# cita-cloud/consensus_overlord

Hardware: AMD Instinct MI355X
Metric: BLS12-381 vote verifications/sec (batch 4096) at 1/2/4/8 MI355X vs host blst (higher is better)
Workload: dtype u32; 1 GPU; config3: 4096 distinct-message precommit votes per GPU, RLC batch verify; batch_per_gpu=4096, global_batch=4096, parallelism=single GPU

## Files before the change

### consensus_overlord_amd/_lib.py

```python
from __future__ import annotations

import ctypes
import os

_HERE = os.path.dirname(os.path.abspath(__file__))
LIB_PATH = os.environ.get("OVH_LIBPATH") or os.path.join(_HERE, "libovhip.so")

_u8p = ctypes.c_char_p
_sz = ctypes.c_size_t
_szp = ctypes.POINTER(ctypes.c_size_t)
_vp = ctypes.c_void_p

SIGNATURES = [
    ("ovh_create", _vp, [ctypes.c_int, _u8p, _sz, ctypes.c_uint32]),
    ("ovh_create_multi", _vp, [ctypes.POINTER(ctypes.c_int), ctypes.c_int, _u8p, _sz, ctypes.c_uint32]),
    ("ovh_multi_peer_matrix", ctypes.c_int, [_vp, _u8p, _sz]),
    ("ovh_destroy", None, [_vp]),
    ("ovh_device_count", ctypes.c_int, [_vp]),
    ("ovh_stream", _vp, [_vp]),
    ("ovh_sm3", ctypes.c_int, [_u8p, _sz, _u8p]),
    ("ovh_sm3_batch", ctypes.c_int, [_vp, _sz, _vp, _vp, _vp]),
    ("ovh_sm3_batch_device", ctypes.c_int, [_vp, _sz, _vp, _vp, _vp]),
    ("ovh_check_blocks", ctypes.c_int, [_vp, _sz, _vp, _vp, _vp, _vp, _vp, _vp, _vp]),
    ("ovh_vote_digests_device", ctypes.c_int, [_vp, _sz, _vp, _vp, _vp, _vp, _vp, _vp]),
# ... 21 lines not shown
    ("ovh_verify_batch_device", ctypes.c_int, [_vp, _sz, _vp, _vp, _vp, _vp]),
    ("ovh_batch_partial_device", ctypes.c_int, [_vp, _sz, _vp, _vp, _vp, _vp, _vp, _vp]),
    ("ovh_combine_partials_device", ctypes.c_int, [_vp, _sz, _vp, ctypes.POINTER(ctypes.c_int32)]),
    ("ovh_batch_fallback_device", ctypes.c_int, [_vp, _sz, _vp]),
    ("ovh_verify_batch_device_async", ctypes.c_int, [_vp, _sz, _vp, _vp, _vp, _vp]),
    ("ovh_verify_samemsg_device_async", ctypes.c_int, [_vp, _sz, _vp, _vp, _vp, _vp]),
    ("ovh_vote_spans", ctypes.c_int, [_vp, ctypes.POINTER(ctypes.c_float), _sz]),
    ("ovh_verify_batch_async", ctypes.c_int, [_vp, _sz, _vp, _vp, _vp, _vp]),
    ("ovh_batch_wait", ctypes.c_int, [_vp]),
    ("ovh_combine_partials_device_async", ctypes.c_int, [_vp, _sz, _vp, _sz, _vp, _vp]),
    ("ovh_stage_times", ctypes.c_int, [_vp, ctypes.POINTER(ctypes.c_float), _sz]),
    ("ovh_stage_name", ctypes.c_char_p, [ctypes.c_int]),
    ("ovh_vm_trace", ctypes.c_int, [_vp, ctypes.c_int, ctypes.POINTER(ctypes.c_uint64), _sz]),
    ("ovh_vm_clock", ctypes.c_int, [_vp, ctypes.POINTER(ctypes.c_uint64), _sz]),
    ("ovh_pool_log", ctypes.c_int, [_vp, ctypes.POINTER(ctypes.c_uint64), _sz]),
    ("ovh_diag_vm_occupancy", ctypes.c_int, [_vp, ctypes.c_int, _sz, ctypes.c_int, ctypes.c_int,
                                             ctypes.POINTER(ctypes.c_float)]),
    ("ovh_sign_batch_device", ctypes.c_int, [_vp, _sz, _vp, _vp, _vp]),
    ("ovh_sk_to_pk_batch_device", ctypes.c_int, [_vp, _sz, _vp, _vp]),
]

_lib = None


def load():
    global _lib
    if _lib is not None:
        return _lib
    if not os.path.exists(LIB_PATH):
        raise RuntimeError(
# ... 13 lines not shown
```

### consensus_overlord_amd/csrc/ovhip.hip

```cpp
#include <hip/hip_runtime.h>

#include <errno.h>
#include <stdlib.h>
#include <sys/random.h>
#include <sys/types.h>

#include <algorithm>
#include <atomic>
#include <deque>
#include <mutex>
#include <new>
#include <string>
#include <string.h>
#include <unordered_map>
#include <vector>

#include "../../include/ovhip.h"
#include "bls/verify.hpp"
#include "fpvm.hpp"
#include "keygen.hpp"
#include "proof.hpp"
#include "qc_segments.hpp"
#include "rlp.hpp"
#include "sm3.hpp"
#include "sm3_bulk.hpp"
#ifdef OVH_VM_PROGS
#include OVH_VM_PROGS
#else
#include <vm_progs.inc>
#endif
static_assert(VM_KZERO == ovh::vm::KZERO && VM_KTAB == ovh::vm::KTAB, "fixed constants (tools/fpvm/gen.py)");
#define VM_ASSERT_NO_INV(P) static_assert(!VM_##P##_HAS_INV, #P " has an inv op: it needs vm::run<SIDE, true>")
#define VM_ASSERT_INV(P) static_assert(VM_##P##_HAS_INV, #P " has no inv op: bind it to vm::run<SIDE, false>")
VM_ASSERT_NO_INV(MADD); VM_ASSERT_NO_INV(PADD); VM_ASSERT_NO_INV(G1PADD);
VM_ASSERT_NO_INV(HDBL1); VM_ASSERT_NO_INV(HDBL2); VM_ASSERT_NO_INV(HDBL4); VM_ASSERT_NO_INV(HDBL8); VM_ASSERT_NO_INV(HDBL16);
// ... 264 lines not shown
};

#define POOL_SEQR 16u
#define POOL_QW 16u
enum : uint32_t {
  PQ_CUR = 0,
  PQ_NPUB = POOL_QW,
  PQ_SLOTOF = 2 * POOL_QW,
  PQ_NANN = 3 * POOL_QW,
  PQ_DONE = 4 * POOL_QW,
  PQ_CLAIM = PQ_DONE + OVH_BATCH_SLOTS * POOL_QW,
  PQ_INFL = PQ_CLAIM + OVH_BATCH_SLOTS * POOL_QW,
  PQ_OCC = PQ_INFL + POOL_QW,
};
constexpr uint32_t POOL_OCC_N = 4096;
constexpr uint32_t PQ_WORDS = PQ_OCC + POOL_OCC_N / 2;
static_assert(POOL_SEQR > OVH_BATCH_SLOTS && POOL_SEQR / 2 <= POOL_QW, "pool queue layout");
#define POOL_IDLE_TICKS 2000ull
#define POOL_WAIT_TICKS 2000000ull

__device__ __forceinline__ uint32_t simd_key() {
  const uint32_t hw = __builtin_amdgcn_s_getreg((31 << 11) | 4);
  const uint32_t xcc = __builtin_amdgcn_s_getreg((3 << 11) | 20);
  return (xcc & 7u) << 9 | ((hw >> 13) & 3u) << 7 | ((hw >> 12) & 1u) << 6 | ((hw >> 8) & 15u) << 2 |
         ((hw >> 4) & 3u);
}
__device__ __forceinline__ uint32_t* pq_occ(uint64_t* q) { return reinterpret_cast<uint32_t*>(q + PQ_OCC); }
#define POOL_SPREAD_TICKS 20000ull

struct PoolBatch {
  uint64_t seq;
  uint32_t n, nq;
  uint32_t table;
  uint32_t has_idx;
  uint64_t seed, base;
  int32_t* codes;
  const uint32_t* planes;
  const uint32_t* flags;
  uint32_t pcap, cap;
  uint32_t* state;
  uint32_t* part0;
  const uint8_t* stage;
// ... 30 lines not shown
}

struct PoolArgs {
  uint64_t* q;
  const PoolBatch* descs;
  const uint4* pv_code;
  const uint32_t* pv_side;
  const uint4* pt_code;
  const uint32_t* pt_side;
  const uint4* fold_code;
  const uint32_t* cst;
  uint32_t* scr;
  uint64_t* wlog;
  uint64_t only;
  uint32_t nsimd;
  uint32_t skip_cu;
};

__device__ __forceinline__ uint64_t* pq_done(uint64_t* q, uint32_t slot) { return q + PQ_DONE + slot * POOL_QW; }
__device__ __forceinline__ uint64_t* pq_claim(uint64_t* q, uint32_t slot) { return q + PQ_CLAIM + slot * POOL_QW; }
__device__ __forceinline__ uint32_t* pq_slot_of(uint64_t* q) { return reinterpret_cast<uint32_t*>(q + PQ_SLOTOF); }
__device__ __forceinline__ uint64_t qld(const uint64_t* p) {
  return __hip_atomic_load(p, __ATOMIC_RELAXED, __HIP_MEMORY_SCOPE_AGENT);
}

__global__ __launch_bounds__(64) void k_pool_publish(PoolBatch b, uint32_t slot, uint64_t seq, uint64_t* q,
                                                     PoolBatch* descs) {
  if (threadIdx.x) return;
  b.seq = ~0ull;
  descs[slot] = b;
  __builtin_amdgcn_fence(__ATOMIC_RELEASE, "agent");
// ... 282 lines not shown
    pl[16 + 2 * quad] = pl_start | (uint64_t)simd_key() << 48 | (uint64_t)how << 60;
    pl[16 + 2 * quad + 1] = __builtin_amdgcn_s_memrealtime();
  }
  __builtin_amdgcn_fence(__ATOMIC_RELEASE, "agent");
  asm volatile("s_waitcnt vmcnt(0)" ::: "memory");
  if (threadIdx.x == 0) {
    __hip_atomic_fetch_add(pq_done(a.q, slot), 1ull, __ATOMIC_RELAXED, __HIP_MEMORY_SCOPE_AGENT);
    __hip_atomic_fetch_add(a.q + PQ_INFL, ~0ull, __ATOMIC_RELAXED, __HIP_MEMORY_SCOPE_AGENT);
    __hip_atomic_fetch_add(pq_occ(a.q) + simd_key(), ~0u, __ATOMIC_RELAXED, __HIP_MEMORY_SCOPE_AGENT);
  }
}

__global__ __launch_bounds__(64, 2) void k_vm_pool(PoolArgs a) {
  __builtin_amdgcn_s_setprio(2);
  extern __shared__ uint4 lds4[];
  if (a.skip_cu && ((simd_key() >> 2) & 0x7Fu) < a.skip_cu) return;
  uint32_t* lds = reinterpret_cast<uint32_t*>(lds4);
  load_consts(lds, a.cst, VM_NCONST);
  const uint64_t t_in = __builtin_amdgcn_s_memrealtime();
  vote_stagger();
  uint32_t nquads = 0, why = 0;
#pragma unroll 1
  for (;; ++nquads) {
    uint32_t slot = 0, quad = 0, how = 0;
    if (!pool_claim(a.q, a.descs, &slot, &quad, &why, a.only, a.nsimd, &how)) break;
    slot = uni(slot);
    quad = uni(quad) | uni(how) << 28;
    __builtin_amdgcn_fence(__ATOMIC_ACQUIRE, "agent");
    vote_quad(a, slot, quad, lds, uni(dget(&a.descs[slot].table)) != 0);
  }
  if (a.wlog && threadIdx.x == 0 && blockIdx.x < PLOG_WGS) {
    uint64_t* w = a.wlog + (size_t)blockIdx.x * PLOG_WG_WORDS;
    w[0] = t_in;
    w[1] = __builtin_amdgcn_s_memrealtime();
    w[2] = nquads;
    w[3] = why;
  }
}

__global__ __launch_bounds__(64) void k_pool_wait(uint64_t* q, uint32_t slot, uint32_t nq, uint64_t ticks,
                                                  uint32_t* err) {
  if (threadIdx.x) return;
  const uint64_t t0 = wall_clock64();
  while (__hip_atomic_load(pq_done(q, slot), __ATOMIC_RELAXED, __HIP_MEMORY_SCOPE_AGENT) < nq) {
    if (wall_clock64() - t0 > ticks) {
      __hip_atomic_store(err, 1u, __ATOMIC_RELAXED, __HIP_MEMORY_SCOPE_SYSTEM);
      return;
    }
    __builtin_amdgcn_s_sleep(32);
  }
}

// ... 1377 lines not shown
struct ovh_ctx {
  int device = 0;
  uint32_t flags = 0;
  hipStream_t stream = nullptr;
  hipStream_t fstream = nullptr, fstream2 = nullptr, fstream3 = nullptr;
  hipStream_t fstream4 = nullptr;
  uint32_t nfin = NFIN_STREAMS;
  hipStream_t xstream = nullptr;
  hipStream_t vstream[3] = {};
  hipStream_t hstream[4] = {};
  hipStream_t pool_st[3] = {};
  uint64_t* pool_q = nullptr;
  void* pool_desc = nullptr;
  uint32_t* pool_scr = nullptr;
  uint32_t pool_wgs = 0;
  uint32_t pool_grid0 = 0;
  uint32_t ncu = 256;
  uint32_t pool_rsv = 0;
  uint32_t pool_ncu = 256;
  uint64_t pool_seq = 0;
  uint32_t* pool_err = nullptr;
  uint64_t* plog = nullptr;
  uint64_t plog_seq[OVH_BATCH_SLOTS] = {};
  uint64_t plog_grids = 0;
  hipStream_t fs[OVH_BATCH_SLOTS] = {};
  hipEvent_t ev_front[OVH_BATCH_SLOTS] = {}, ev_back[OVH_BATCH_SLOTS] = {};
  hipEvent_t ev_x[4] = {};
  uint32_t* state_slot[OVH_BATCH_SLOTS] = {};
  uint32_t* red_slot[OVH_BATCH_SLOTS] = {};
  uint32_t *state_all = nullptr, *red_all = nullptr;
  uint8_t* pstage_all = nullptr;
  size_t state_w = 0, red_w = 0, pstage_b = 0;
  int32_t* grp_ok[OVH_BATCH_SLOTS] = {};
  uint32_t slot_n[OVH_BATCH_SLOTS] = {};
// ... 125 lines not shown
static_assert(LDS_VSAME8 <= 64 * 1024, "vsame8 LDS (default limit)");
static constexpr size_t LDS_H2G = ((size_t)SLOT_BASE_W + VM_SLICES * (size_t)H2G_STRIDE_W) * 4;
static constexpr size_t LDS_GMIL = ((size_t)SLOT_BASE_W + (size_t)VM_GMIL_NSLOTS * 12) * 4;
static_assert(LDS_VSAME <= 64 * 1024 && LDS_H2G <= 64 * 1024 && LDS_GMIL + 16 <= 64 * 1024, "same-message LDS");
static constexpr size_t LDS_PKDEC = ((size_t)SLOT_BASE_W + (64 / VM_PKDEC_W) * (size_t)PKDEC_STRIDE_W) * 4;
static_assert(LDS_PKDEC <= 64 * 1024 && VM_PKDEC_NIN == 2, "pkdec LDS / shape");
static constexpr size_t LDS_G1GRP = ((size_t)SLOT_BASE_W + (size_t)G1GRP_STRIDE_W) * 4;
static_assert(LDS_G1GRP <= 64 * 1024 && VM_G1GRP_NIN == 3, "g1grp LDS / shape");
static constexpr size_t LDS_GFIN = ((size_t)SLOT_BASE_W + (size_t)VM_GFIN_NSLOTS * 12) * 4;
static_assert(LDS_GFIN + 16 <= 64 * 1024, "gfin LDS");
constexpr size_t lds_granule(size_t b) { return (b + 1023) / 1024 * 1024; }
static constexpr size_t LDS_POOL = LDS_VOTE > LDS_VOTE_T ? LDS_VOTE : LDS_VOTE_T;
static_assert(8 * lds_granule(LDS_POOL) <= 160 * 1024, "eight pool workgroups per CU");
static_assert(VOTE_NSCR <= 4096 && VM_VOTE_NSLOTS <= 2048 && VM_VOTE_T_NSLOTS <= 2048,
              "side words: 12-bit scratch entries, 11-bit slots (fpvm.hpp side_spill)");
#ifndef POOL_HOLES_PER_8CU
#define POOL_HOLES_PER_8CU 8u
#endif
#define POOL_MAX_WGS 4096u
static_assert(FOLD_STRIDE_W <= VM_SLICES * VOTE_STRIDE_W && FOLD_STRIDE_W <= VM_SLICES * VOTE_T_STRIDE_W,
              "fused fold reuses the vote slots");

static int vm_upload(ovh_ctx* c, VmDev& d, const uint32_t* code, uint32_t nphases, uint32_t W, uint32_t NW,
                     const uint16_t* in, uint32_t nin, const uint16_t* out, uint32_t nout,
                     const uint32_t* side = nullptr) {
  const size_t words = (size_t)nphases * W * NW, pad = (size_t)vm::PREFETCH * W * NW;
  void *dc = nullptr, *di = nullptr, *dout = nullptr;
  HIPCHK(hipMalloc(&dc, (words + pad) * 4));
  c->vm_bufs.push_back(dc);
  HIPCHK(hipMemcpy(dc, code, words * 4, hipMemcpyHostToDevice));
  HIPCHK(hipMemset((uint32_t*)dc + words, 0, pad * 4));
  HIPCHK(hipMalloc(&di, nin * 2 + 2));
// ... 144 lines not shown
};

static const uint8_t DEFAULT_DST[] = "BLS_SIG_BLS12381G2_XMD:SHA-256_SSWU_RO_NUL_";

static uint32_t nblk(size_t n) { return (uint32_t)((n + WG - 1) / WG); }

static Slab region_F(ovh_ctx* c, int slot, int r) {
  return Slab{c->red_slot[slot] + (size_t)r * PART_PLANES * 12 * c->red_cap, c->red_cap};
}
static Slab region_S(ovh_ctx* c, int slot, int r) {
  return Slab{c->red_slot[slot] + (size_t)r * PART_PLANES * 12 * c->red_cap + (size_t)12 * 12 * c->red_cap,
              c->red_cap};
}

namespace {
struct ParkedStream {
  int device;
  int prio;
  hipStream_t s;
};
std::mutex g_park_mu;
std::vector<ParkedStream> g_parked;
}

static hipError_t stream_new(hipStream_t* s, int prio) {
  int dev = 0;
  const hipError_t e = hipGetDevice(&dev);
  if (e != hipSuccess) return e;
  {
    std::lock_guard<std::mutex> g(g_park_mu);
    for (size_t k = 0; k < g_parked.size(); ++k)
      if (g_parked[k].device == dev && g_parked[k].prio == prio) {
        *s = g_parked[k].s;
        g_parked.erase(g_parked.begin() + (ptrdiff_t)k);
        return hipSuccess;
      }
  }
  return hipStreamCreateWithPriority(s, hipStreamNonBlocking, prio);
}

static void stream_park(int device, hipStream_t s) {
  if (!s) return;
  (void)hipStreamSynchronize(s);
  int prio = 0;
  if (hipStreamGetPriority(s, &prio) != hipSuccess) return;
  std::lock_guard<std::mutex> g(g_park_mu);
  g_parked.push_back(ParkedStream{device, prio, s});
}

static int pool_failed(const ovh_ctx* c) {
  return c->pool_err && __atomic_load_n(c->pool_err, __ATOMIC_ACQUIRE) ? OVH_ERR_DEVICE : 0;
}

static int sync_all(ovh_ctx* c) {
  HIPCHK(hipStreamSynchronize(c->stream));
  HIPCHK(hipStreamSynchronize(c->fstream));
  HIPCHK(hipStreamSynchronize(c->fstream2));
  HIPCHK(hipStreamSynchronize(c->fstream3));
  if (c->fstream4) HIPCHK(hipStreamSynchronize(c->fstream4));
  for (hipStream_t s : {c->pool_st[0], c->pool_st[1], c->pool_st[2], c->vstream[0], c->vstream[1], c->vstream[2],
                        c->hstream[1], c->hstream[2], c->hstream[3]})
    if (s) HIPCHK(hipStreamSynchronize(s));
// ... 180 lines not shown
  b.part_cap = r0.cap;
  b.stage = ps;
  b.clk = table ? c->vm_vote_t.clk : c->vm_vote.clk;
  b.plog = c->plog ? c->plog + (size_t)(seq % PLOG_RING) * PLOG_WORDS : nullptr;
  c->plog_seq[slot] = seq;
  k_pool_publish<<<1, 64, 0, c->stream>>>(b, (uint32_t)slot, seq, c->pool_q, (PoolBatch*)c->pool_desc);
  if (b.plog) k_stamp<<<1, 64, 0, c->stream>>>(b.plog + PLOG_EV_PUB, seq);
  HIPCHK(hipEventRecord(c->ev_front[slot], c->stream));
  c->slot_n[slot] = n;
  c->last_n = n;
  const bool vev = (c->flags & OVH_FLAG_PROFILE) != 0;
  const uint32_t vk = c->vev_n % ovh_ctx::VEV_CAP;
  const uint32_t wgs = c->pool_wgs;
  PoolArgs pa;
  pa.only = ~0ull;
  pa.nsimd = 4 * c->pool_ncu;
  pa.skip_cu = c->pool_rsv / 8;
  shard = shard && !c->pool_rsv;
  pa.q = c->pool_q;
  pa.descs = (const PoolBatch*)c->pool_desc;
  pa.pv_code = c->vm_vote.code;
  pa.pv_side = c->vm_vote.side;
  pa.pt_code = c->vm_vote_t.code;
  pa.pt_side = c->vm_vote_t.side;
  pa.fold_code = c->vm_fold.code;
  pa.cst = c->vm_consts;
  for (uint32_t par = 0; launch && par < (shard ? c->shard_streams : 2u); ++par) {
    if (shard && par != (uint32_t)(seq % c->shard_streams)) continue;
    if (shard) pa.only = seq + c->shard_span;
    hipStream_t pst = c->pool_st[par];
    HIPCHK(hipStreamWaitEvent(pst, c->ev_front[slot], 0));
    if (par == 0 || shard) {
      if (c->flags & OVH_FLAG_PROFILE) HIPCHK(hipEventRecord(c->ev0[ST_VOTE], pst));
      if (vev) HIPCHK(hipEventRecord(c->vev0[vk], pst));
    }
    const uint32_t gw = shard ? 2 * wgs : par == 0 ? c->pool_grid0 : 2 * wgs - c->pool_grid0;
    pa.scr = c->pool_scr + (size_t)par * 2 * wgs * VM_SLICES * VOTE_NSCR * 12;
    pa.wlog = nullptr;
    if (c->plog) {
      uint64_t* g = c->plog + PLOG_GRID_BASE + (size_t)(c->plog_grids++ % PLOG_GRIDS) * (4 + PLOG_WGS * PLOG_WG_WORDS);
      k_grid_hdr<<<1, 64, 0, pst>>>(g, seq, par, gw);
      pa.wlog = g + 4;
    }
    k_vm_pool<<<gw, 64, LDS_POOL, pst>>>(pa);
    if (par == 1 || shard) {
      if (c->flags & OVH_FLAG_PROFILE) {
        HIPCHK(hipEventRecord(c->ev1[ST_VOTE], pst));
        c->ev_mask |= 1u << ST_VOTE;
      }
      if (vev) {
        HIPCHK(hipEventRecord(c->vev1[vk], pst));
// ... 403 lines not shown
  const uint32_t* head = pl.head;
  const uint32_t* pairs = pl.pairs;
  c->ev_mask = 0;
  uint64_t seed, base;
  CHK(draw_seed(c, &seed, &base));
  c->slot_seed[slot] = seed;
  c->slot_base[slot] = base;
  const hipStream_t fst = c->fs[slot];
  hipStream_t st = c->stream;
  if (one) {
    hipStream_t* pair = c->vstream;
    for (hipStream_t* v : {&pair[0], &pair[1]})
      if (!*v) {
        int lo = 0, hi = 0;
        (void)hipDeviceGetStreamPriorityRange(&lo, &hi);
        HIPCHK(stream_new(v, hi));
      }
    st = pair[c->pipe_k & 1];
  }
  if (!c->xstream) HIPCHK(stream_new(&c->xstream, 0));
  const uint32_t hk = one ? (uint32_t)(c->pipe_k % SM_H2G_STREAMS) : 0u;
  if (hk && !c->hstream[hk]) HIPCHK(stream_new(&c->hstream[hk], 0));
  const hipStream_t xs = one ? fst : c->xstream, hs = hk ? c->hstream[hk] : c->xstream;
  HIPCHK(hipEventRecord(c->ev_front[slot], c->stream));
  HIPCHK(hipStreamWaitEvent(hs, c->ev_front[slot], 0));
  HIPCHK(hipStreamWaitEvent(fst, c->ev_front[slot], 0));
  if (st != c->stream) HIPCHK(hipStreamWaitEvent(st, c->ev_front[slot], 0));
  {
    StageScope p(c, ST_H2F, hs);
    if (one) k_put_hash<<<1, 64, 0, hs>>>(*one, (uint8_t*)ghash);
    k_h2f<<<nblk(G), WG, 0, hs>>>(G, ghash, c->xmd, g);
    k_vm_h2g<<<(G + VM_SLICES - 1) / VM_SLICES, 64, LDS_H2G, hs>>>(G, c->vm_h2g, c->vm_consts, g, ghinf);
  }
  HIPCHK(hipEventRecord(c->ev_x[1], hs));
  HIPCHK(hipStreamWaitEvent(fst, c->ev_x[1], 0));
  const PkSrc tab{c->tab.planes, c->tab.cap, c->tab.flags, tidx};
  {
// ... 509 lines not shown
  if (!c) return nullptr;
  c->device = device;
  c->flags = flags;
  if (const char* e = getenv("OVH_SMALL_MAX")) c->small_max = (uint32_t)atoi(e);
  if (const char* e = getenv("OVH_SAMEMSG")) c->samemsg = atoi(e);
  if (const char* e = getenv("OVH_SHARD_SPAN")) c->shard_span = (uint32_t)atoi(e);
  if (const char* e = getenv("OVH_SHARD_STREAMS")) c->shard_streams = atoi(e) == 3 ? 3u : 2u;
  if (const char* e = getenv("OVH_NFIN")) c->nfin = atoi(e) == 3 ? 3u : atoi(e) == 2 ? 2u : NFIN_STREAMS;
  int ncu = 0;
  if (hipDeviceGetAttribute(&ncu, hipDeviceAttributeMultiprocessorCount, device) != hipSuccess || ncu <= 0) ncu = 256;
  if (flags & OVH_FLAG_POOL_RESERVE) {
    c->pool_rsv = 8;
    if (const char* e = getenv("OVH_POOL_RESERVE")) c->pool_rsv = (uint32_t)atoi(e);
    if (c->pool_rsv % 8 || c->pool_rsv > 64 || (uint32_t)ncu <= 2 * c->pool_rsv) c->pool_rsv = 0;
  }
  const uint32_t pncu = (uint32_t)ncu - c->pool_rsv;
  uint32_t holes = POOL_HOLES_PER_8CU;
  if (const char* e = c->pool_rsv ? getenv("OVH_POOL_PER_CU") : nullptr) holes = atoi(e) == 8 ? 0u : holes;
  c->pool_wgs = ((uint32_t)ncu * 8 - (uint32_t)ncu * holes / 8) / 2;
  if (c->pool_wgs > POOL_MAX_WGS) c->pool_wgs = POOL_MAX_WGS;
  c->pool_grid0 = std::min(4u * (uint32_t)ncu, 2 * c->pool_wgs - 1);
  c->ncu = (uint32_t)ncu;
  c->pool_ncu = pncu;
  if (!dst) {
    dst = DEFAULT_DST;
    dst_len = 43;
  }
  int lo = 0, hi = 0;
  (void)hipDeviceGetStreamPriorityRange(&lo, &hi);
  bool ok = xmd_build_templates(c->xmd, dst, dst_len) &&
            stream_new(&c->stream, 0) == hipSuccess &&
            stream_new(&c->fstream, lo) == hipSuccess &&
            stream_new(&c->fstream2, lo) == hipSuccess &&
            stream_new(&c->fstream3, lo) == hipSuccess &&
            (c->nfin < 4 || stream_new(&c->fstream4, lo) == hipSuccess) &&
            stream_new(&c->pool_st[0], hi) == hipSuccess &&
            stream_new(&c->pool_st[1], hi) == hipSuccess &&
            (c->shard_streams < 3 || stream_new(&c->pool_st[2], hi) == hipSuccess) &&
            hipMalloc(&c->part_out, (size_t)OVH_BATCH_SLOTS * 2 * 216 * 4) == hipSuccess && hipMalloc(&c->result, RES_WORDS * 4) == hipSuccess &&
            hipMemset(c->result, 0, RES_WORDS * 4) == hipSuccess &&
            hipMalloc(&c->pool_q, (size_t)PQ_WORDS * 8) == hipSuccess && hipMemset(c->pool_q, 0, (size_t)PQ_WORDS * 8) == hipSuccess &&
            hipMalloc(&c->pool_desc, sizeof(PoolBatch) * OVH_BATCH_SLOTS) == hipSuccess &&
            hipMemset(c->pool_desc, 0, sizeof(PoolBatch) * OVH_BATCH_SLOTS) == hipSuccess &&
            hipMalloc(&c->pool_scr, (size_t)2 * c->shard_streams * c->pool_wgs * VM_SLICES * VOTE_NSCR * 48) == hipSuccess &&
            hipHostMalloc((void**)&c->pool_err, 64, hipHostMallocCoherent | hipHostMallocMapped) == hipSuccess &&
            hipMalloc(&c->fin, (size_t)OVH_BATCH_SLOTS * FIN_STRIDE * 4) == hipSuccess && vm_init(c) == 0;
  if (ok) *c->pool_err = 0;
  if (ok && (flags & OVH_FLAG_VM_CLOCK))
    ok = hipMalloc(&c->plog, PLOG_TOTAL * 8) == hipSuccess && hipMemset(c->plog, 0, PLOG_TOTAL * 8) == hipSuccess;
  ok = ok && hipDeviceSynchronize() == hipSuccess;
  for (int k = 0; ok && k < OVH_BATCH_SLOTS; ++k) c->fs[k] = c->fstream;
  for (int k = 0; ok && k < OVH_BATCH_SLOTS; ++k)
    ok = hipEventCreateWithFlags(&c->ev_front[k], hipEventDisableTiming) == hipSuccess &&
         hipEventCreateWithFlags(&c->ev_back[k], hipEventDisableTiming) == hipSuccess;
  for (int k = 0; ok && k < 4; ++k) ok = hipEventCreateWithFlags(&c->ev_x[k], hipEventDisableTiming) == hipSuccess;
  for (int k = 0; ok && k < OVH_BATCH_SLOTS; ++k)
// ... 93 lines not shown
  for (int k = 0; k < OVH_BATCH_SLOTS; ++k) {
    for (int q = 0; q < 4; ++q)
      if (c->ev_m[k][q]) (void)hipEventDestroy(c->ev_m[k][q]);
    if (c->hst_h[k]) (void)hipHostFree(c->hst_h[k]);
    if (c->hst_d[k]) (void)hipFree(c->hst_d[k]);
  }
  if (c->mg) (void)hipFree(c->mg);
  for (int k = 0; k < OVH_NSTAGES; ++k) {
    if (c->ev0[k]) (void)hipEventDestroy(c->ev0[k]);
    if (c->ev1[k]) (void)hipEventDestroy(c->ev1[k]);
  }
  for (uint32_t k = 0; k < ovh_ctx::VEV_CAP; ++k) {
    if (c->vev0[k]) (void)hipEventDestroy(c->vev0[k]);
    if (c->vev1[k]) (void)hipEventDestroy(c->vev1[k]);
  }
  for (hipStream_t s : {c->stream, c->fstream, c->fstream2, c->fstream3, c->fstream4, c->xstream, c->vstream[0], c->vstream[1], c->vstream[2],
                        c->pool_st[0], c->pool_st[1], c->pool_st[2], c->hstream[1], c->hstream[2], c->hstream[3]})
    stream_park(c->device, s);
  if (c->pool_err) (void)hipHostFree(c->pool_err);
  delete c;
}

void ovh_destroy(ovh_ctx* c) {
  if (!c) return;
  for (ovh_ctx* s : c->sub) destroy_one(s);
  c->sub.clear();
  destroy_one(c);
}

int ovh_device_count(ovh_ctx* c) { return !c ? 0 : c->sub.empty() ? 1 : (int)c->sub.size(); }

int ovh_diag_vm_occupancy(ovh_ctx* c, int prog, size_t n, int reps, int streams, float* ms) {
  if (!c || !ms || n == 0 || n > (1u << 20) || reps < 1 || streams < 1 || streams > 2 || prog < 0 || prog > 2 ||
      (prog == 2 && reps > OVH_BATCH_SLOTS))
    return OVH_ERR_ARG;
  if (!c->sub.empty()) c = c->sub[0];
  std::lock_guard<std::mutex> g(c->mu);
  HIPCHK(hipSetDevice(c->device));
  CHK(ensure_cap(c, n));
  CHK(ensure_in(c, n * 180 + 64));
  CHK(sync_all(c));
  if (!c->xstream) HIPCHK(stream_new(&c->xstream, 0));
  HIPCHK(hipMemsetAsync(c->in_buf, 0, n * 180, c->stream));
  HIPCHK(hipStreamSynchronize(c->stream));
  const Slab s{c->state_slot[0], c->cap};
  int32_t* dc = (int32_t*)(c->in_buf + n * 176);
  const uint32_t N = (uint32_t)n;
  hipEvent_t e0, e1;
  HIPCHK(hipEventCreate(&e0));
  HIPCHK(hipEventCreate(&e1));
  HIPCHK(hipEventRecord(e0, c->stream));
  HIPCHK(hipStreamWaitEvent(c->xstream, e0, 0));
  for (int r = 0; r < reps; ++r) {
    if (prog == 0) {
      hipStream_t st = (streams == 2 && (r & 1)) ? c->xstream : c->stream;
      k_vm_vsame<false><<<(N + VM_SLICES - 1) / VM_SLICES, 64, LDS_VSAME, st>>>(N, 0, c->vm_vsame, c->vm_consts,
                                                                               c->in_buf + n * 128, PkSrc{}, c->in_buf,
// ... 43 lines not shown
  if (hipSetDevice(c->device) != hipSuccess || sync_all(c)) return -OVH_ERR_DEVICE;
  const VmDev* d = c->clk_table ? &c->vm_vote_t : &c->vm_vote;
  const size_t n = (size_t)2 * c->clk_wgs, k = max < n ? max : n;
  if (k && hipMemcpy(stamps, d->clk, k * 8, hipMemcpyDeviceToHost) != hipSuccess) return -OVH_ERR_DEVICE;
  return (int)n;
}

int ovh_pool_log(ovh_ctx* c, uint64_t* words, size_t max) {
  if (!c || (max && !words)) return -OVH_ERR_ARG;
  if (!c->sub.empty()) c = c->sub[0];
  if (!c->plog) return 0;
  std::lock_guard<std::mutex> g(c->mu);
  if (hipSetDevice(c->device) != hipSuccess || sync_all(c)) return -OVH_ERR_DEVICE;
  const size_t n = PLOG_TOTAL, k = max < n ? max : n;
  if (k && hipMemcpy(words, c->plog, k * 8, hipMemcpyDeviceToHost) != hipSuccess) return -OVH_ERR_DEVICE;
  return (int)n;
}

int ovh_stage_times(ovh_ctx* c, float* ms, size_t max) {
  if (!c || (!ms && max)) return -OVH_ERR_ARG;
  if (!c->sub.empty()) c = c->sub[0];
  if (!(c->flags & OVH_FLAG_PROFILE)) return 0;
  std::lock_guard<std::mutex> g(c->mu);
  if (hipSetDevice(c->device) != hipSuccess || sync_all(c)) return -OVH_ERR_DEVICE;
  const size_t n = max < OVH_NSTAGES ? max : OVH_NSTAGES;
  for (size_t k = 0; k < n; ++k) {
    ms[k] = 0.f;
    if (c->ev_mask & (1u << k))
      if (hipEventElapsedTime(&ms[k], c->ev0[k], c->ev1[k]) != hipSuccess) return -OVH_ERR_DEVICE;
  }
// ... 261 lines not shown
  CHK(stage_list(c, sigs, sig_lens, n, 0, &ds, &so, &sl, &used1));
  CHK(stage_list(c, pks, pk_lens, n, used1, &dp, &po, &pl, &used2));
  if (n && !compressed) {
    uint8_t* cs = c->in_buf + ((used2 + 15) & ~(size_t)15);
    uint64_t* co = (uint64_t*)(cs + (size_t)96 * n);
    k_canon_sig_list<<<nblk(n), WG, 0, c->stream>>>((uint32_t)n, ds, so, sl, cs, co);
    HIPCHK(hipGetLastError());
    ds = cs;
    so = co;
    used2 = (size_t)((uint8_t*)(co + n) - c->in_buf);
  }
  Slab pts{c->scr, c->scr_cap};
  Slab ppts{c->scr + (size_t)6 * 12 * c->scr_cap, c->scr_cap};
  if (n) {
    HIPCHK(hipEventRecord(c->ev_x[2], c->stream));
    if (!c->xstream) HIPCHK(stream_new(&c->xstream, 0));
    HIPCHK(hipStreamWaitEvent(c->xstream, c->ev_x[2], 0));
    bool keys48 = true;
    for (size_t i = 0; i < n; ++i) keys48 = keys48 && pk_lens[i] == 48;
    if (keys48) {
      constexpr uint32_t KSL = 64 / VM_PKDEC_W;
      k_vm_pkdec<<<(uint32_t)((n + KSL - 1) / KSL), 64, LDS_PKDEC, c->xstream>>>((uint32_t)n, c->vm_pkdec,
                                                                                c->vm_consts, dp, po, c->scr_pk);
    } else {
      k_parse_pk_list<<<nblk(n), WG, 0, c->xstream>>>((uint32_t)n, dp, po, pl, c->scr_pk, ppts);
    }
    HIPCHK(hipGetLastError());
    HIPCHK(hipEventRecord(c->ev_x[3], c->xstream));
    const int gc = (c->flags & OVH_FLAG_AGG_NO_GROUPCHECK) ? 0 : 1;
    constexpr uint32_t SL = 64 / VM_SIGCHK_W;
    k_vm_sigchk<<<(uint32_t)((n + SL - 1) / SL), 64, LDS_SIGCHK, c->stream>>>((uint32_t)n, c->vm_sigchk, c->vm_consts,
// ... 171 lines not shown
    uint8_t* dp;
    uint64_t *po, *pl;
    size_t used = 0;
    CHK(stage_list(c, pks, pk_lens, n, raw_base, &dp, &po, &pl, &used));
    uint8_t* rs = c->in_buf + used;
    if (agg_len) HIPCHK(hipMemcpyAsync(rs, agg_sig, agg_len, hipMemcpyHostToDevice, c->stream));
    k_canon_qc<<<nblk(n + 1), WG, 0, c->stream>>>((uint32_t)n, dp, po, pl, rs, (uint32_t)agg_len, d);
    HIPCHK(hipGetLastError());
  }
  HIPCHK(hipMemcpyAsync(d + n * 48 + 96, hash, 32, hipMemcpyHostToDevice, c->stream));
  int slot;
  CHK(take_slot(c, &slot));
  c->last_n = 0;
  Slab s{c->state_slot[slot], c->cap};
  HIPCHK(hipEventRecord(c->ev_x[2], c->stream));
  if (!c->xstream) HIPCHK(stream_new(&c->xstream, 0));
  HIPCHK(hipStreamWaitEvent(c->xstream, c->ev_x[2], 0));
  k_h2f<<<1, WG, 0, c->xstream>>>(1, d + n * 48 + 96, c->xmd, s);
  k_vm_qcpre<<<1, 64, LDS_QCPRE, c->xstream>>>(c->vm_qcpre, c->vm_consts, d + n * 48, s, qpf);
  HIPCHK(hipGetLastError());
  HIPCHK(hipEventRecord(c->ev_x[3], c->xstream));
  uint32_t* kflags = c->qt_buf + (size_t)3 * 12 * c->qt_cap;
  constexpr uint32_t PK_SL = 64 / VM_PKCHK_W;
  k_vm_pkchk<<<(uint32_t)((n + PK_SL - 1) / PK_SL), 64, LDS_PKCHK, c->stream>>>((uint32_t)n, c->vm_pkchk, c->vm_consts, d,
                                                                               Slab{c->qt_buf, c->qt_cap}, kflags);
  HIPCHK(hipGetLastError());
  std::vector<uint32_t> hf(n);
  HIPCHK(hipMemcpyAsync(hf.data(), kflags, n * 4, hipMemcpyDeviceToHost, c->stream));
  HIPCHK(hipStreamSynchronize(c->stream));
  uint32_t fl = 0;
  for (size_t i = 0; i < n; ++i) fl |= hf[i];
// ... 1062 lines not shown
```

### include/ovhip.h

```cpp
#ifndef OVHIP_H
#define OVHIP_H

#include <stddef.h>
#include <stdint.h>

#ifdef __cplusplus
extern "C" {
#endif

typedef struct ovh_ctx ovh_ctx;

#define OVH_OK 0
#define OVH_ERR_HASH_LEN 100
#define OVH_ERR_LEN_MISMATCH 101
#define OVH_ERR_PUBKEY 102
#define OVH_ERR_ARG 103
#define OVH_ERR_DEVICE 200
#define OVH_ERR_RNG 201

#define OVH_FLAG_AGG_NO_GROUPCHECK 0x1u
#define OVH_FLAG_PROFILE 0x2u
#define OVH_FLAG_VM_TRACE 0x4u
#define OVH_FLAG_TEST_RLC 0x8u
#define OVH_FLAG_SK_RAW 0x10u
// ... 86 lines not shown
int ovh_verify_batch_async(ovh_ctx* ctx, size_t n, const uint8_t* sigs, const uint8_t* hashes, const uint8_t* pks,
                           int32_t* codes);
int ovh_batch_wait(ovh_ctx* ctx);
int ovh_combine_partials_device_async(ovh_ctx* ctx, size_t k, const uint8_t* d_partials, size_t n,
                                      int32_t* d_codes, void* stream);

int ovh_stage_times(ovh_ctx* ctx, float* ms, size_t max);
const char* ovh_stage_name(int stage);
int ovh_vote_spans(ovh_ctx* ctx, float* ms, size_t max);

int ovh_vm_trace(ovh_ctx* ctx, int prog, uint64_t* stamps, size_t max);
int ovh_diag_vm_occupancy(ovh_ctx* ctx, int prog, size_t n, int reps, int streams, float* ms);
int ovh_vm_clock(ovh_ctx* ctx, uint64_t* stamps, size_t max);

int ovh_pool_log(ovh_ctx* ctx, uint64_t* words, size_t max);

int ovh_sign_batch_device(ovh_ctx* ctx, size_t n, const uint8_t* d_sks, const uint8_t* d_hashes, uint8_t* d_sigs);
int ovh_sk_to_pk_batch_device(ovh_ctx* ctx, size_t n, const uint8_t* d_sks, uint8_t* d_pks);

#ifdef __cplusplus
}
#endif

#endif
```

### overlord-hip/build.rs

```rust
use std::{env, path::PathBuf, process::Command};

fn main() {
    let manifest = PathBuf::from(env::var("CARGO_MANIFEST_DIR").unwrap());
    let src = env::var("OVHIP_SRC")
        .map(PathBuf::from)
        .unwrap_or_else(|_| manifest.join("../consensus_overlord_amd"));
    assert!(
        src.join("csrc/ovhip.hip").exists(),
        "libovhip sources not found at {} (set OVHIP_SRC)",
        src.display()
    );
    let hipcc = env::var("HIPCC").unwrap_or_else(|_| "/opt/rocm/bin/hipcc".into());
    let arch = env::var("OVHIP_ARCH").unwrap_or_else(|_| "gfx950".into());
    let out = PathBuf::from(env::var("OUT_DIR").unwrap());

    let gen = Command::new("python3")
        .arg(src.join("../tools/fpvm/gen.py"))
        .arg("--out")
        .arg(out.join("vm_progs.inc"))
        .status()
        .expect("python3 (tools/fpvm/gen.py)");
    assert!(gen.success(), "tools/fpvm/gen.py failed");

    let st = Command::new(&hipcc)
        .args(["-O3", "-std=c++17", "-fPIC", "-Wno-unused-result", "-shared"])
        .arg(format!("--offload-arch={arch}"))
        .arg(format!("-I{}", out.display()))
        .arg("-o")
        .arg(out.join("libovhip.so"))
        .arg(src.join("csrc/ovhip.hip"))
        .status()
        .expect("hipcc");
    assert!(st.success(), "hipcc --offload-arch={arch} failed");

    println!("cargo:rustc-link-search=native={}", out.display());
    println!("cargo:rustc-link-lib=dylib=ovhip");
    println!("cargo:rustc-link-arg=-Wl,-rpath,{}", out.display());
    for f in ["csrc/ovhip.hip", "csrc/fpvm.hpp", "csrc/msm.hpp", "csrc/keygen.hpp", "csrc/rlp.hpp", "csrc/sm3.hpp", "csrc/sm3_bulk.hpp", "csrc/proof.hpp", "csrc/qc.hpp", "csrc/bls"] {
        println!("cargo:rerun-if-changed={}", src.join(f).display());
    }
    println!("cargo:rerun-if-changed={}", src.join("../include/ovhip.h").display());
    println!("cargo:rerun-if-changed={}", src.join("../tools/fpvm").display());
    println!("cargo:rerun-if-env-changed=OVHIP_SRC");
    println!("cargo:rerun-if-env-changed=HIPCC");
    println!("cargo:rerun-if-env-changed=OVHIP_ARCH");
}
```

### overlord-hip/src/ffi.rs

```rust
#![allow(non_camel_case_types)]
use std::os::raw::{c_char, c_void};

#[repr(C)]
pub struct OvhCtx {
    _p: [u8; 0],
}

pub const OVH_OK: i32 = 0;
pub const OVH_ERR_HASH_LEN: i32 = 100;
pub const OVH_ERR_LEN_MISMATCH: i32 = 101;
pub const OVH_ERR_PUBKEY: i32 = 102;
pub const OVH_ERR_ARG: i32 = 103;
pub const OVH_ERR_DEVICE: i32 = 200;
pub const OVH_ERR_RNG: i32 = 201;
pub const OVH_CB_PROOF_DECODE: i32 = 300;
pub const OVH_CB_MISMATCH: i32 = 301;

pub const OVH_FLAG_AGG_NO_GROUPCHECK: u32 = 0x1;
pub const OVH_FLAG_PROFILE: u32 = 0x2;
pub const OVH_FLAG_VM_TRACE: u32 = 0x4;
pub const OVH_FLAG_TEST_RLC: u32 = 0x8;
pub const OVH_FLAG_SK_RAW: u32 = 0x10;
pub const OVH_FLAG_VM_CLOCK: u32 = 0x20;
pub const OVH_FLAG_POOL_RESERVE: u32 = 0x40;
// ... 39 lines not shown
    pub fn ovh_batch_partial_device(ctx: *mut OvhCtx, n: usize, d_sigs: *const u8, d_hashes: *const u8, d_pks: *const u8, d_codes: *mut i32, d_partial: *mut u8, stream: *mut c_void) -> i32;
    pub fn ovh_combine_partials_device(ctx: *mut OvhCtx, k: usize, d_partials: *const u8, verdict: *mut i32) -> i32;
    pub fn ovh_batch_fallback_device(ctx: *mut OvhCtx, n: usize, d_codes: *mut i32) -> i32;
    pub fn ovh_verify_batch_device_async(ctx: *mut OvhCtx, n: usize, d_sigs: *const u8, d_hashes: *const u8, d_pks: *const u8, d_codes: *mut i32) -> i32;
    pub fn ovh_verify_samemsg_device_async(ctx: *mut OvhCtx, n: usize, d_sigs: *const u8, hash: *const u8, d_pks: *const u8, d_codes: *mut i32) -> i32;
    pub fn ovh_verify_batch_async(ctx: *mut OvhCtx, n: usize, sigs: *const u8, hashes: *const u8, pks: *const u8, codes: *mut i32) -> i32;
    pub fn ovh_batch_wait(ctx: *mut OvhCtx) -> i32;
    pub fn ovh_combine_partials_device_async(ctx: *mut OvhCtx, k: usize, d_partials: *const u8, n: usize, d_codes: *mut i32, stream: *mut c_void) -> i32;
    pub fn ovh_stage_times(ctx: *mut OvhCtx, ms: *mut f32, max: usize) -> i32;
    pub fn ovh_stage_name(stage: i32) -> *const c_char;
    pub fn ovh_vote_spans(ctx: *mut OvhCtx, ms: *mut f32, max: usize) -> i32;
    pub fn ovh_vm_trace(ctx: *mut OvhCtx, prog: i32, stamps: *mut u64, max: usize) -> i32;
    pub fn ovh_diag_vm_occupancy(ctx: *mut OvhCtx, prog: i32, n: usize, reps: i32, streams: i32, ms: *mut f32) -> i32;
    pub fn ovh_vm_clock(ctx: *mut OvhCtx, stamps: *mut u64, max: usize) -> i32;
    pub fn ovh_pool_log(ctx: *mut OvhCtx, words: *mut u64, max: usize) -> i32;
    pub fn ovh_sign_batch_device(ctx: *mut OvhCtx, n: usize, d_sks: *const u8, d_hashes: *const u8, d_sigs: *mut u8) -> i32;
    pub fn ovh_sk_to_pk_batch_device(ctx: *mut OvhCtx, n: usize, d_sks: *const u8, d_pks: *mut u8) -> i32;
}
```

Baseline: 1.806 million verifications/s.

## Admit pool workgroups per CU via device-side admission limits instead of holes

Replaces the old scheme, which shrank the pool grid by a fixed number of holes per 8 CUs and skipped reserved CUs, with a per-CU admission table in device memory. Each pool workgroup atomically claims a slot on its CU and exits if the CU's limit (7 or 8 by pattern, 0 for reserved CUs) is reached. The grid is now sized for a full 8 workgroups per CU, and the effective SIMD count is reduced by a reserve counter. The aim is finer control over per-CU occupancy for the persistent VM pool, at the cost of extra atomics at kernel entry and exit. Stream parking is also rekeyed by role instead of priority, and a diagnostic getter for the admission table is added.

```diff
diff --git a/consensus_overlord_amd/_lib.py b/consensus_overlord_amd/_lib.py
--- a/consensus_overlord_amd/_lib.py
+++ b/consensus_overlord_amd/_lib.py
@@ -59,6 +59,7 @@
     ("ovh_vm_trace", ctypes.c_int, [_vp, ctypes.c_int, ctypes.POINTER(ctypes.c_uint64), _sz]),
     ("ovh_vm_clock", ctypes.c_int, [_vp, ctypes.POINTER(ctypes.c_uint64), _sz]),
     ("ovh_pool_log", ctypes.c_int, [_vp, ctypes.POINTER(ctypes.c_uint64), _sz]),
+    ("ovh_pool_admission", ctypes.c_int, [_vp, ctypes.POINTER(ctypes.c_uint32), _sz]),
     ("ovh_diag_vm_occupancy", ctypes.c_int, [_vp, ctypes.c_int, _sz, ctypes.c_int, ctypes.c_int,
                                              ctypes.POINTER(ctypes.c_float)]),
     ("ovh_sign_batch_device", ctypes.c_int, [_vp, _sz, _vp, _vp, _vp]),
diff --git a/consensus_overlord_amd/csrc/ovhip.hip b/consensus_overlord_amd/csrc/ovhip.hip
--- a/consensus_overlord_amd/csrc/ovhip.hip
+++ b/consensus_overlord_amd/csrc/ovhip.hip
@@ -19,6 +19,7 @@
 #include "bls/verify.hpp"
 #include "fpvm.hpp"
 #include "keygen.hpp"
+#include "pool_admit.hpp"
 #include "proof.hpp"
 #include "qc_segments.hpp"
 #include "rlp.hpp"
@@ -313,7 +314,10 @@
   PQ_OCC = PQ_INFL + POOL_QW,
 };
 constexpr uint32_t POOL_OCC_N = 4096;
-constexpr uint32_t PQ_WORDS = PQ_OCC + POOL_OCC_N / 2;
+constexpr uint32_t PQ_RSV = PQ_OCC + POOL_OCC_N / 2;
+constexpr uint32_t PQ_CU = PQ_RSV + POOL_QW;
+constexpr uint32_t PQ_WORDS = PQ_CU + pool_admit::CU_KEYS;
+constexpr uint32_t POOL_LIMIT_SEEN = 0x100u;
 static_assert(POOL_SEQR > OVH_BATCH_SLOTS && POOL_SEQR / 2 <= POOL_QW, "pool queue layout");
 #define POOL_IDLE_TICKS 2000ull
 #define POOL_WAIT_TICKS 2000000ull
@@ -325,6 +329,7 @@
          ((hw >> 4) & 3u);
 }
 __device__ __forceinline__ uint32_t* pq_occ(uint64_t* q) { return reinterpret_cast<uint32_t*>(q + PQ_OCC); }
+__device__ __forceinline__ uint32_t* pq_cu(uint64_t* q) { return reinterpret_cast<uint32_t*>(q + PQ_CU); }
 #define POOL_SPREAD_TICKS 20000ull
 
 struct PoolBatch {
@@ -385,7 +390,6 @@
   uint64_t* wlog;
   uint64_t only;
   uint32_t nsimd;
-  uint32_t skip_cu;
 };
 
 __device__ __forceinline__ uint64_t* pq_done(uint64_t* q, uint32_t slot) { return q + PQ_DONE + slot * POOL_QW; }
@@ -698,16 +702,28 @@
 __global__ __launch_bounds__(64, 2) void k_vm_pool(PoolArgs a) {
   __builtin_amdgcn_s_setprio(2);
   extern __shared__ uint4 lds4[];
-  if (a.skip_cu && ((simd_key() >> 2) & 0x7Fu) < a.skip_cu) return;
+  uint32_t* const res = pq_cu(a.q) + (simd_key() >> 2);
+  const uint32_t lim = __builtin_amdgcn_readfirstlane(
+      __hip_atomic_load(res + pool_admit::CU_KEYS, __ATOMIC_RELAXED, __HIP_MEMORY_SCOPE_AGENT));
+  if (lane0_fetch_add32(res, 1u) >= (lim & 0xFFu)) {
+    if (threadIdx.x == 0) {
+      __hip_atomic_fetch_add(res, ~0u, __ATOMIC_RELAXED, __HIP_MEMORY_SCOPE_AGENT);
+      if (lim == 0 && !(__hip_atomic_fetch_or(res + pool_admit::CU_KEYS, POOL_LIMIT_SEEN, __ATOMIC_RELAXED,
+                                              __HIP_MEMORY_SCOPE_AGENT) & POOL_LIMIT_SEEN))
+        __hip_atomic_fetch_add(a.q + PQ_RSV, 4ull, __ATOMIC_RELAXED, __HIP_MEMORY_SCOPE_AGENT);
+    }
+    return;
+  }
   uint32_t* lds = reinterpret_cast<uint32_t*>(lds4);
   load_consts(lds, a.cst, VM_NCONST);
   const uint64_t t_in = __builtin_amdgcn_s_memrealtime();
   vote_stagger();
   uint32_t nquads = 0, why = 0;
+  const uint32_t nsimd = a.nsimd - (uint32_t)qldu(a.q + PQ_RSV);
 #pragma unroll 1
   for (;; ++nquads) {
     uint32_t slot = 0, quad = 0, how = 0;
-    if (!pool_claim(a.q, a.descs, &slot, &quad, &why, a.only, a.nsimd, &how)) break;
+    if (!pool_claim(a.q, a.descs, &slot, &quad, &why, a.only, nsimd, &how)) break;
     slot = uni(slot);
     quad = uni(quad) | uni(how) << 28;
     __builtin_amdgcn_fence(__ATOMIC_ACQUIRE, "agent");
@@ -720,6 +736,8 @@
     w[2] = nquads;
     w[3] = why;
   }
+  if (threadIdx.x == 0)
+    __hip_atomic_fetch_add(pq_cu(a.q) + (simd_key() >> 2), ~0u, __ATOMIC_RELAXED, __HIP_MEMORY_SCOPE_AGENT);
 }
 
 __global__ __launch_bounds__(64) void k_pool_wait(uint64_t* q, uint32_t slot, uint32_t nq, uint64_t ticks,
@@ -2127,10 +2145,10 @@
   void* pool_desc = nullptr;
   uint32_t* pool_scr = nullptr;
   uint32_t pool_wgs = 0;
-  uint32_t pool_grid0 = 0;
+  uint32_t pool_grid0 = 0, pool_grid1 = 0;
   uint32_t ncu = 256;
   uint32_t pool_rsv = 0;
-  uint32_t pool_ncu = 256;
+  uint32_t pool_pattern = 0;
   uint64_t pool_seq = 0;
   uint32_t* pool_err = nullptr;
   uint64_t* plog = nullptr;
@@ -2286,8 +2304,8 @@
 static_assert(8 * lds_granule(LDS_POOL) <= 160 * 1024, "eight pool workgroups per CU");
 static_assert(VOTE_NSCR <= 4096 && VM_VOTE_NSLOTS <= 2048 && VM_VOTE_T_NSLOTS <= 2048,
               "side words: 12-bit scratch entries, 11-bit slots (fpvm.hpp side_spill)");
-#ifndef POOL_HOLES_PER_8CU
-#define POOL_HOLES_PER_8CU 8u
+#ifndef POOL_PATTERN_DEFAULT
+#define POOL_PATTERN_DEFAULT 0u
 #endif
 #define POOL_MAX_WGS 4096u
 static_assert(FOLD_STRIDE_W <= VM_SLICES * VOTE_STRIDE_W && FOLD_STRIDE_W <= VM_SLICES * VOTE_T_STRIDE_W,
@@ -2462,23 +2480,25 @@
 }
 
 namespace {
+enum StreamRole : int { SR_MAIN, SR_FIN, SR_FIN2, SR_FIN3, SR_FIN4, SR_X, SR_V0, SR_V1, SR_V2, SR_POOL0, SR_POOL1, SR_POOL2,
+                        SR_H1, SR_H2, SR_H3 };
 struct ParkedStream {
   int device;
-  int prio;
+  int role;
   hipStream_t s;
 };
 std::mutex g_park_mu;
 std::vector<ParkedStream> g_parked;
 }
 
-static hipError_t stream_new(hipStream_t* s, int prio) {
+static hipError_t stream_new(hipStream_t* s, int prio, int role) {
   int dev = 0;
   const hipError_t e = hipGetDevice(&dev);
   if (e != hipSuccess) return e;
   {
     std::lock_guard<std::mutex> g(g_park_mu);
     for (size_t k = 0; k < g_parked.size(); ++k)
-      if (g_parked[k].device == dev && g_parked[k].prio == prio) {
+      if (g_parked[k].device == dev && g_parked[k].role == role) {
         *s = g_parked[k].s;
         g_parked.erase(g_parked.begin() + (ptrdiff_t)k);
         return hipSuccess;
@@ -2487,13 +2507,11 @@
   return hipStreamCreateWithPriority(s, hipStreamNonBlocking, prio);
 }
 
-static void stream_park(int device, hipStream_t s) {
+static void stream_park(int device, hipStream_t s, int role) {
   if (!s) return;
   (void)hipStreamSynchronize(s);
-  int prio = 0;
-  if (hipStreamGetPriority(s, &prio) != hipSuccess) return;
   std::lock_guard<std::mutex> g(g_park_mu);
-  g_parked.push_back(ParkedStream{device, prio, s});
+  g_parked.push_back(ParkedStream{device, role, s});
 }
 
 static int pool_failed(const ovh_ctx* c) {
@@ -2704,8 +2722,7 @@
   const uint32_t wgs = c->pool_wgs;
   PoolArgs pa;
   pa.only = ~0ull;
-  pa.nsimd = 4 * c->pool_ncu;
-  pa.skip_cu = c->pool_rsv / 8;
+  pa.nsimd = 4 * c->ncu;
   shard = shard && !c->pool_rsv;
   pa.q = c->pool_q;
   pa.descs = (const PoolBatch*)c->pool_desc;
@@ -2724,7 +2741,7 @@
       if (c->flags & OVH_FLAG_PROFILE) HIPCHK(hipEventRecord(c->ev0[ST_VOTE], pst));
       if (vev) HIPCHK(hipEventRecord(c->vev0[vk], pst));
     }
-    const uint32_t gw = shard ? 2 * wgs : par == 0 ? c->pool_grid0 : 2 * wgs - c->pool_grid0;
+    const uint32_t gw = shard ? 2 * wgs : par == 0 ? c->pool_grid0 : c->pool_grid1;
     pa.scr = c->pool_scr + (size_t)par * 2 * wgs * VM_SLICES * VOTE_NSCR * 12;
     pa.wlog = nullptr;
     if (c->plog) {
@@ -3158,13 +3175,13 @@
       if (!*v) {
         int lo = 0, hi = 0;
         (void)hipDeviceGetStreamPriorityRange(&lo, &hi);
-        HIPCHK(stream_new(v, hi));
+        HIPCHK(stream_new(v, hi, SR_V0 + (int)(v - pair)));
       }
     st = pair[c->pipe_k & 1];
   }
-  if (!c->xstream) HIPCHK(stream_new(&c->xstream, 0));
+  if (!c->xstream) HIPCHK(stream_new(&c->xstream, 0, SR_X));
   const uint32_t hk = one ? (uint32_t)(c->pipe_k % SM_H2G_STREAMS) : 0u;
-  if (hk && !c->hstream[hk]) HIPCHK(stream_new(&c->hstream[hk], 0));
+  if (hk && !c->hstream[hk]) HIPCHK(stream_new(&c->hstream[hk], 0, SR_H1 + (int)hk - 1));
   const hipStream_t xs = one ? fst : c->xstream, hs = hk ? c->hstream[hk] : c->xstream;
   HIPCHK(hipEventRecord(c->ev_front[slot], c->stream));
   HIPCHK(hipStreamWaitEvent(hs, c->ev_front[slot], 0));
@@ -3704,14 +3721,18 @@
     if (const char* e = getenv("OVH_POOL_RESERVE")) c->pool_rsv = (uint32_t)atoi(e);
     if (c->pool_rsv % 8 || c->pool_rsv > 64 || (uint32_t)ncu <= 2 * c->pool_rsv) c->pool_rsv = 0;
   }
-  const uint32_t pncu = (uint32_t)ncu - c->pool_rsv;
-  uint32_t holes = POOL_HOLES_PER_8CU;
-  if (const char* e = c->pool_rsv ? getenv("OVH_POOL_PER_CU") : nullptr) holes = atoi(e) == 8 ? 0u : holes;
-  c->pool_wgs = ((uint32_t)ncu * 8 - (uint32_t)ncu * holes / 8) / 2;
+  c->pool_pattern = POOL_PATTERN_DEFAULT;
+  if (const char* e = getenv("OVH_POOL_PATTERN")) c->pool_pattern = (uint32_t)atoi(e) < pool_admit::PATTERNS ? (uint32_t)atoi(e) : c->pool_pattern;
+  uint8_t lim8[pool_admit::CU_KEYS];
+  pool_admit::limits(c->pool_pattern, c->pool_rsv / 8, lim8);
+  if (const char* e = c->pool_rsv ? getenv("OVH_POOL_PER_CU") : nullptr)
+    for (uint8_t& l : lim8) l = atoi(e) == 8 && l ? 8 : l;
+  std::vector<uint32_t> lim(lim8, lim8 + pool_admit::CU_KEYS);
+  c->pool_wgs = (uint32_t)ncu * 8u / 2;
   if (c->pool_wgs > POOL_MAX_WGS) c->pool_wgs = POOL_MAX_WGS;
   c->pool_grid0 = std::min(4u * (uint32_t)ncu, 2 * c->pool_wgs - 1);
+  c->pool_grid1 = 2 * c->pool_wgs - c->pool_grid0;
   c->ncu = (uint32_t)ncu;
-  c->pool_ncu = pncu;
   if (!dst) {
     dst = DEFAULT_DST;
     dst_len = 43;
@@ -3719,17 +3740,18 @@
   int lo = 0, hi = 0;
   (void)hipDeviceGetStreamPriorityRange(&lo, &hi);
   bool ok = xmd_build_templates(c->xmd, dst, dst_len) &&
-            stream_new(&c->stream, 0) == hipSuccess &&
-            stream_new(&c->fstream, lo) == hipSuccess &&
-            stream_new(&c->fstream2, lo) == hipSuccess &&
-            stream_new(&c->fstream3, lo) == hipSuccess &&
-            (c->nfin < 4 || stream_new(&c->fstream4, lo) == hipSuccess) &&
-            stream_new(&c->pool_st[0], hi) == hipSuccess &&
-            stream_new(&c->pool_st[1], hi) == hipSuccess &&
-            (c->shard_streams < 3 || stream_new(&c->pool_st[2], hi) == hipSuccess) &&
+            stream_new(&c->stream, 0, SR_MAIN) == hipSuccess &&
+            stream_new(&c->fstream, lo, SR_FIN) == hipSuccess &&
+            stream_new(&c->fstream2, lo, SR_FIN2) == hipSuccess &&
+            stream_new(&c->fstream3, lo, SR_FIN3) == hipSuccess &&
+            (c->nfin < 4 || stream_new(&c->fstream4, lo, SR_FIN4) == hipSuccess) &&
+            stream_new(&c->pool_st[0], hi, SR_POOL0) == hipSuccess &&
+            stream_new(&c->pool_st[1], hi, SR_POOL1) == hipSuccess &&
+            (c->shard_streams < 3 || stream_new(&c->pool_st[2], hi, SR_POOL2) == hipSuccess) &&
             hipMalloc(&c->part_out, (size_t)OVH_BATCH_SLOTS * 2 * 216 * 4) == hipSuccess && hipMalloc(&c->result, RES_WORDS * 4) == hipSuccess &&
             hipMemset(c->result, 0, RES_WORDS * 4) == hipSuccess &&
             hipMalloc(&c->pool_q, (size_t)PQ_WORDS * 8) == hipSuccess && hipMemset(c->pool_q, 0, (size_t)PQ_WORDS * 8) == hipSuccess &&
+            hipMemcpy(reinterpret_cast<uint32_t*>(c->pool_q + PQ_CU) + pool_admit::CU_KEYS, lim.data(), pool_admit::CU_KEYS * 4, hipMemcpyHostToDevice) == hipSuccess &&
             hipMalloc(&c->pool_desc, sizeof(PoolBatch) * OVH_BATCH_SLOTS) == hipSuccess &&
             hipMemset(c->pool_desc, 0, sizeof(PoolBatch) * OVH_BATCH_SLOTS) == hipSuccess &&
             hipMalloc(&c->pool_scr, (size_t)2 * c->shard_streams * c->pool_wgs * VM_SLICES * VOTE_NSCR * 48) == hipSuccess &&
@@ -3853,9 +3875,10 @@
     if (c->vev0[k]) (void)hipEventDestroy(c->vev0[k]);
     if (c->vev1[k]) (void)hipEventDestroy(c->vev1[k]);
   }
-  for (hipStream_t s : {c->stream, c->fstream, c->fstream2, c->fstream3, c->fstream4, c->xstream, c->vstream[0], c->vstream[1], c->vstream[2],
-                        c->pool_st[0], c->pool_st[1], c->pool_st[2], c->hstream[1], c->hstream[2], c->hstream[3]})
-    stream_park(c->device, s);
+  const hipStream_t by_role[] = {c->stream, c->fstream, c->fstream2, c->fstream3, c->fstream4, c->xstream, c->vstream[0],
+                                 c->vstream[1], c->vstream[2], c->pool_st[0], c->pool_st[1], c->pool_st[2], c->hstream[1],
+                                 c->hstream[2], c->hstream[3]};
+  for (int r = 0; r <= SR_H3; ++r) stream_park(c->device, by_role[r], r);
   if (c->pool_err) (void)hipHostFree(c->pool_err);
   delete c;
 }
@@ -3879,7 +3902,7 @@
   CHK(ensure_cap(c, n));
   CHK(ensure_in(c, n * 180 + 64));
   CHK(sync_all(c));
-  if (!c->xstream) HIPCHK(stream_new(&c->xstream, 0));
+  if (!c->xstream) HIPCHK(stream_new(&c->xstream, 0, SR_X));
   HIPCHK(hipMemsetAsync(c->in_buf, 0, n * 180, c->stream));
   HIPCHK(hipStreamSynchronize(c->stream));
   const Slab s{c->state_slot[0], c->cap};
@@ -3953,6 +3976,16 @@
   if (hipSetDevice(c->device) != hipSuccess || sync_all(c)) return -OVH_ERR_DEVICE;
   const size_t n = PLOG_TOTAL, k = max < n ? max : n;
   if (k && hipMemcpy(words, c->plog, k * 8, hipMemcpyDeviceToHost) != hipSuccess) return -OVH_ERR_DEVICE;
+  return (int)n;
+}
+
+int ovh_pool_admission(ovh_ctx* c, uint32_t* words, size_t max) {
+  if (!c || (max && !words)) return -OVH_ERR_ARG;
+  if (!c->sub.empty()) c = c->sub[0];
+  std::lock_guard<std::mutex> g(c->mu);
+  if (hipSetDevice(c->device) != hipSuccess || sync_all(c)) return -OVH_ERR_DEVICE;
+  const size_t n = (size_t)2 * pool_admit::CU_KEYS, k = max < n ? max : n;
+  if (k && hipMemcpy(words, c->pool_q + PQ_CU, k * 4, hipMemcpyDeviceToHost) != hipSuccess) return -OVH_ERR_DEVICE;
   return (int)n;
 }
 
@@ -4244,7 +4277,7 @@
   Slab ppts{c->scr + (size_t)6 * 12 * c->scr_cap, c->scr_cap};
   if (n) {
     HIPCHK(hipEventRecord(c->ev_x[2], c->stream));
-    if (!c->xstream) HIPCHK(stream_new(&c->xstream, 0));
+    if (!c->xstream) HIPCHK(stream_new(&c->xstream, 0, SR_X));
     HIPCHK(hipStreamWaitEvent(c->xstream, c->ev_x[2], 0));
     bool keys48 = true;
     for (size_t i = 0; i < n; ++i) keys48 = keys48 && pk_lens[i] == 48;
@@ -4446,7 +4479,7 @@
   c->last_n = 0;
   Slab s{c->state_slot[slot], c->cap};
   HIPCHK(hipEventRecord(c->ev_x[2], c->stream));
-  if (!c->xstream) HIPCHK(stream_new(&c->xstream, 0));
+  if (!c->xstream) HIPCHK(stream_new(&c->xstream, 0, SR_X));
   HIPCHK(hipStreamWaitEvent(c->xstream, c->ev_x[2], 0));
   k_h2f<<<1, WG, 0, c->xstream>>>(1, d + n * 48 + 96, c->xmd, s);
   k_vm_qcpre<<<1, 64, LDS_QCPRE, c->xstream>>>(c->vm_qcpre, c->vm_consts, d + n * 48, s, qpf);
diff --git a/consensus_overlord_amd/csrc/pool_admit.hpp b/consensus_overlord_amd/csrc/pool_admit.hpp
--- /dev/null
+++ b/consensus_overlord_amd/csrc/pool_admit.hpp
@@ -0,0 +1,40 @@
+#pragma once
+#include <cstdint>
+
+namespace pool_admit {
+
+constexpr uint32_t CU_KEYS = 1024;
+constexpr uint32_t CU_IDS = 16;
+constexpr uint32_t PATTERNS = 4;
+
+constexpr uint32_t period(uint32_t pattern) { return 1u << (pattern < PATTERNS ? pattern : 0u); }
+
+constexpr uint32_t cu_key(uint32_t xcc, uint32_t se, uint32_t sa, uint32_t cu) {
+  return (xcc & 7u) << 7 | (se & 3u) << 5 | (sa & 1u) << 4 | (cu & 15u);
+}
+
+inline void limits(uint32_t pattern, uint32_t rsv_per_xcc, uint8_t out[CU_KEYS]) {
+  const uint32_t per = period(pattern);
+  for (uint32_t k = 0; k < CU_KEYS; ++k) {
+    const uint32_t cu = k & 15u, array = (k >> 4) & 7u;
+    out[k] = cu % per == 0 ? 7 : 8;
+    if (array == 0 && cu < rsv_per_xcc) out[k] = 0;
+  }
+}
+
+inline uint32_t offered(const uint8_t lim[CU_KEYS]) {
+  uint32_t m = 0;
+  for (uint32_t k = 0; k < CU_KEYS; ++k) m = lim[k] > m ? lim[k] : m;
+  return m;
+}
+
+inline uint32_t admitted(const uint8_t lim[CU_KEYS], uint32_t nxcc, uint32_t nse, uint32_t nsa, uint32_t cus) {
+  uint32_t n = 0;
+  for (uint32_t x = 0; x < nxcc; ++x)
+    for (uint32_t e = 0; e < nse; ++e)
+      for (uint32_t a = 0; a < nsa; ++a)
+        for (uint32_t c = 0; c < cus && c < CU_IDS; ++c) n += lim[cu_key(x, e, a, c)];
+  return n;
+}
+
+}
diff --git a/include/ovhip.h b/include/ovhip.h
--- a/include/ovhip.h
+++ b/include/ovhip.h
@@ -124,6 +124,7 @@
 int ovh_vm_clock(ovh_ctx* ctx, uint64_t* stamps, size_t max);
 
 int ovh_pool_log(ovh_ctx* ctx, uint64_t* words, size_t max);
+int ovh_pool_admission(ovh_ctx* ctx, uint32_t* words, size_t max);
 
 int ovh_sign_batch_device(ovh_ctx* ctx, size_t n, const uint8_t* d_sks, const uint8_t* d_hashes, uint8_t* d_sigs);
 int ovh_sk_to_pk_batch_device(ovh_ctx* ctx, size_t n, const uint8_t* d_sks, uint8_t* d_pks);
diff --git a/overlord-hip/build.rs b/overlord-hip/build.rs
--- a/overlord-hip/build.rs
+++ b/overlord-hip/build.rs
@@ -36,7 +36,7 @@
     println!("cargo:rustc-link-search=native={}", out.display());
     println!("cargo:rustc-link-lib=dylib=ovhip");
     println!("cargo:rustc-link-arg=-Wl,-rpath,{}", out.display());
-    for f in ["csrc/ovhip.hip", "csrc/fpvm.hpp", "csrc/msm.hpp", "csrc/keygen.hpp", "csrc/rlp.hpp", "csrc/sm3.hpp", "csrc/sm3_bulk.hpp", "csrc/proof.hpp", "csrc/qc.hpp", "csrc/bls"] {
+    for f in ["csrc/ovhip.hip", "csrc/fpvm.hpp", "csrc/msm.hpp", "csrc/keygen.hpp", "csrc/pool_admit.hpp", "csrc/rlp.hpp", "csrc/sm3.hpp", "csrc/sm3_bulk.hpp", "csrc/proof.hpp", "csrc/qc.hpp", "csrc/bls"] {
         println!("cargo:rerun-if-changed={}", src.join(f).display());
     }
     println!("cargo:rerun-if-changed={}", src.join("../include/ovhip.h").display());
diff --git a/overlord-hip/src/ffi.rs b/overlord-hip/src/ffi.rs
--- a/overlord-hip/src/ffi.rs
+++ b/overlord-hip/src/ffi.rs
@@ -77,6 +77,7 @@
     pub fn ovh_diag_vm_occupancy(ctx: *mut OvhCtx, prog: i32, n: usize, reps: i32, streams: i32, ms: *mut f32) -> i32;
     pub fn ovh_vm_clock(ctx: *mut OvhCtx, stamps: *mut u64, max: usize) -> i32;
     pub fn ovh_pool_log(ctx: *mut OvhCtx, words: *mut u64, max: usize) -> i32;
+    pub fn ovh_pool_admission(ctx: *mut OvhCtx, words: *mut u32, max: usize) -> i32;
     pub fn ovh_sign_batch_device(ctx: *mut OvhCtx, n: usize, d_sks: *const u8, d_hashes: *const u8, d_sigs: *mut u8) -> i32;
     pub fn ovh_sk_to_pk_batch_device(ctx: *mut OvhCtx, n: usize, d_sks: *const u8, d_pks: *mut u8) -> i32;
 }
```

Result: no change. 1.804 million verifications/s (-0.1%).
